# optimusride/altro-cpp

Measured on AMD Instinct MI355X. Metric: trajectories solved/sec (AL-iLQR to tol), unicycle 101 knots, batched, higher is better.
Workload: dtype f64; 1 GPU; BASELINE configs[2]: batch 4096/GPU unicycle kTurn90 (n=3, m=2, 101 knots), goal + control-bound constraints, full AL loop, default SolverOptions; batch_per_gpu=4096, global_batch=4096, knot_points=101, parallelism=instance-sharded x1 (no data-path collective; RCCL all_gather of result records), device=AMD Radeon Graphics, cus=256

## Files before the change

altro-cpp_amd/csrc/altro_common.hpp:

```cpp
#pragma once

#include <algorithm>
#include <atomic>
#include <cstddef>
#include <initializer_list>
#include <string>
#include <vector>

#include "../../include/altro_hip.h"

namespace altro_hip {

constexpr int kMaxConPerKnot = 4;
constexpr int kMaxClasses = 8;
constexpr int kMaxCostGroups = 8;
#ifndef ALTRO_LS_LANES
#define ALTRO_LS_LANES 20
#endif
constexpr int kLineSearchLanes = ALTRO_LS_LANES;
constexpr int kHistFields = 8;
constexpr int kMaxRuns = 16;
constexpr int kMaxFastCircles = 3;
constexpr int kMaxSharedPool = 128;
constexpr int kParPerKnot = 2;
// ... 366 lines not shown
  ALTRO_HD int total() const { return raw() + fwd_block_pad_bytes((long long)raw() * (long long)sizeof(T)) / (int)sizeof(T); }
};
template <class T>
struct FusedLds {
  FwdLds<T> blk;
  int N, nm, npool;
  static constexpr int kE = (int)sizeof(T), kD = (int)sizeof(double);
  ALTRO_HD int oPool() const { return blk.total() * kE; }
  ALTRO_HD int oXch() const { return oPool() + blk.padv(npool) * kE; }
  ALTRO_HD int oFlags() const { return oXch() + 2 * kSyncFused * nm * kBlock * kE; }
  ALTRO_HD int oGrad() const { return oFlags() + 2 * kBlock * (int)sizeof(int); }
  ALTRO_HD int oFh() const { return oGrad() + kBlock * kD; }
  ALTRO_HD int oJunk() const { return oFh() + kFhWords * kD; }
  ALTRO_HD int oActive() const { return oJunk() + kBlock * kD; }
  ALTRO_HD int oFf() const { return oActive() + 2 * kD; }
  ALTRO_HD int oCand() const { return oFf() + kFfWords * kD; }
  ALTRO_HD int oKD2() const { return oCand() + (N + 1) * kLineSearchLanes * nm * kE; }
  ALTRO_HD int oFh2() const { return oKD2() + (blk.nKD + kBlock) * kE; }
  ALTRO_HD int oAlpha() const { return oFh2() + kFh2Words * kD; }
  ALTRO_HD int oSync() const { return oAlpha() + kLineSearchLanes * kD; }
  ALTRO_HD int oCost() const { return oSync() + kSyWords * (int)sizeof(int); }
  ALTRO_HD int oCvalAhead() const { return oCost() + ((N + 2) & ~1) * kE; }
  ALTRO_HD int used() const { return oCvalAhead() + blk.rowsP() * kE; }
  ALTRO_HD size_t bytes() const { return (size_t)used() + 8 * kD + (size_t)(N + 4 - ((N + 2) & ~1)) * kE; }
};

inline int ChainClaimLocal(int device, int delta) {
  static std::atomic<int> n[64];
  std::atomic<int>& c = n[device >= 0 && device < 64 ? device : 63];
  if (delta == 0) return c.load();
  return c.fetch_add(delta) + delta;
}
using ChainClaimFn = int (*)(int, int);
inline ChainClaimFn& ChainClaimHook() {
  static ChainClaimFn fn = &ChainClaimLocal;
  return fn;
}
inline int ChainClaim(int device, int delta) { return ChainClaimHook()(device, delta); }

class EngineBase {
 public:
  virtual ~EngineBase() {}
  virtual altro_status Upload(const ProblemSpec& spec, std::string* err) = 0;
  virtual altro_status SetInitialState(const ProblemSpec& spec, std::string* err) = 0;
  virtual altro_status SetTrajectory(const ProblemSpec& spec, std::string* err) = 0;
  virtual altro_status SetStep(float hstep) = 0;
// ... 82 lines not shown
```

altro-cpp_amd/csrc/altro_engine.hpp:

```cpp
#pragma once

#include <algorithm>
#include <atomic>
#include <chrono>
#include <cmath>
#include <cstdio>
#include <cstdlib>
#include <cstring>
#include <limits>
#include <map>
#include <string>
#include <thread>
#include <type_traits>
#include <vector>

#include "altro_devmem.hpp"
#include "altro_kernels.hpp"
#include "altro_problem.hpp"

namespace altro_hip {

#define ALTRO_HIP_CHECK(expr)                                                                  \
  do {                                                                                         \
    hipError_t e_ = (expr);                                                                    \
// ... 17 lines not shown
struct Switches {
  struct OptInt {
    bool set = false;
    int v = 0;
  };
  bool poison_on = false;
  unsigned poison_pattern = 0;
  int poison_mix = 0;
  OptInt persist_at;
  bool twin = true;
  bool segments = true;
  OptInt chains;
  OptInt fwd_per_wave;
  int fwd_src = kFwdSrcAuto;
  int sweep_loop = -1;
  OptInt loop_per_cu;
  int cand_front = 6;
  bool twin_debug = false;
  bool twin_debug_all = false;
  int twin_depth = kTwinDefaultDepth;
  int twin_min = tw_min_share(kTwinDefaultMin);
  int twin_spread = kTwinDefaultSpread;
  int twin_misclaim = 0;
  const char* sweep_log = nullptr;
  bool loop_log = false;
  bool force_valu_backward = false, force_coop_backward = false;
  bool dense_expansions = true;
  int spec_mode = kSpecAuto;
  bool fast_forward = false;
  bool begin_merged = true;
  bool no_fused = false;

  static bool NotZero(const char* e) { return !(e && atoi(e) == 0); }
  static bool Is(const char* e, const char* what) { return e && std::strcmp(e, what) == 0; }
  Switches() {
    auto env = [](const char* name) { return std::getenv(name); };
    auto number = [&](const char* name) {
      const char* e = env(name);
      return e ? OptInt{true, atoi(e)} : OptInt{};
    };
    if (const char* e = env("ALTRO_HIP_DEBUG_POISON")) {
      poison_on = true;
      poison_pattern = (unsigned)strtoul(e, nullptr, 16);
      poison_mix = std::strchr(e, ',') != nullptr;
    }
    persist_at = number("ALTRO_HIP_PERSIST_AT");
    twin = NotZero(env("ALTRO_HIP_TWIN"));
    segments = NotZero(env("ALTRO_HIP_SEGMENTS"));
    chains = number("ALTRO_HIP_CHAINS");
    if (chains.set) chains.v = std::max(1, std::min(kMaxSweepChains, chains.v));
    fwd_per_wave = number("ALTRO_HIP_FWD_PER_WAVE");
    if (const char* e = env("ALTRO_HIP_FWD_SRC")) fwd_src = Is(e, "global") ? kFwdSrcGlobal : kFwdSrcOther;
    if (const char* e = env("ALTRO_HIP_SWEEP_LOOP")) sweep_loop = NotZero(e) ? 1 : 0;
    loop_per_cu = number("ALTRO_HIP_LOOP_PER_CU");
    if (const char* e = env("ALTRO_HIP_CAND_FRONT")) cand_front = std::max(0, std::min(kLineSearchLanes - 1, atoi(e)));
    twin_debug = env("ALTRO_HIP_TWIN_DEBUG") != nullptr;
    twin_debug_all = Is(env("ALTRO_HIP_TWIN_DEBUG"), "all");
    if (const char* e = env("ALTRO_HIP_TWIN_DEPTH")) twin_depth = std::max(1, std::min(kTwinMaxDepth, atoi(e)));
    if (const char* e = env("ALTRO_HIP_TWIN_MIN")) twin_min = tw_min_share(atoi(e));
    if (const char* e = env("ALTRO_HIP_TWIN_SPREAD")) twin_spread = std::max(0, std::min(kTwinMaxSpread, atoi(e)));
    if (const char* e = env("ALTRO_HIP_TWIN_MISCLAIM")) twin_misclaim = std::max(0, atoi(e));
    sweep_log = env("ALTRO_HIP_SWEEP_LOG");
    loop_log = env("ALTRO_HIP_LOOP_LOG") != nullptr;
    force_valu_backward = Is(env("ALTRO_HIP_BACKWARD"), "valu");
    force_coop_backward = Is(env("ALTRO_HIP_BACKWARD"), "coop");
    dense_expansions = env("ALTRO_HIP_NO_DENSE_EXPANSIONS") == nullptr;
    const char* spec = env("ALTRO_HIP_SPECULATION");
    spec_mode = Is(spec, "off") ? (int)kSpecOff : Is(spec, "free") ? (int)kSpecFree : Is(spec, "wave") ? (int)kSpecWave : kSpecAuto;
    fast_forward = env("ALTRO_HIP_FAST_FORWARD_STALLS") != nullptr;
    begin_merged = !Is(env("ALTRO_HIP_BEGIN_SOLVE"), "split");
    no_fused = env("ALTRO_HIP_NO_FUSED_SWEEP") != nullptr;
  }
};

inline DevOpts ToDevOpts(const altro_options& o) {
  DevOpts d{};
  d.max_iterations_total = o.max_iterations_total;
  d.max_iterations_outer = o.max_iterations_outer;
  d.max_iterations_inner = o.max_iterations_inner;
  d.bp_reg_fail_threshold = o.bp_reg_fail_threshold;
  d.check_forwardpass_bounds = o.check_forwardpass_bounds;
  d.line_search_max_iterations = o.line_search_max_iterations;
  d.reset_duals = o.reset_duals;
  d.cost_tolerance = o.cost_tolerance;
// ... 2480 lines not shown
        A.act_list = up_.d_merged;
        A.act_count = merged_count;
        timing_.launches += 1;
      }
      A.host_count = nullptr;
      A.next_list = nullptr;
      A.next_count = nullptr;
      PoisonLds();
      if (r.prof) {
        r.fused_ev = r.nev;
        hipEventRecord(ProfEvent(r.nev++), stream_);
      }
      bool circles = false;
      for (int k = 0; k < pd_.nruns; ++k)
        circles = circles || pd_.runs[k].fast == kFastC || pd_.runs[k].fast == kFastCB || pd_.runs[k].fast == kFastBC;
      int* const out = r.loop_launched ? up_.d_loop_ctl + kLwWords : hm_.d_counter.get() + r.max_sweeps + 2;
      const int spec = sw_.spec_mode == kSpecAuto ? (circles ? (int)kSpecWave : (int)kSpecFree) : sw_.spec_mode;
      TwinCtl tw{};
      if (up_.twin_cap > 0 && !A.hist && !r.d.fast_forward_stalls) {
        if (!twin_box_clean_)
          hipMemsetAsync(up_.d_twin_box, 0, TwinBoxWords() * sizeof(unsigned long long), stream_);
        const int min_share = any_split ? std::max(sw_.twin_min, kTwinSegMin) : sw_.twin_min;
        const int pool = std::min(up_.twin_cap, std::max(ninst, num_cus_ - ninst));
        tw = TwinCtl{up_.d_twin_box, up_.d_twin_box + (size_t)2 * up_.twin_cap * kTwWords, ninst, up_.twin_cap, Bp_ - up_.twin_cap, kTwinLag, sw_.twin_debug ? 1 : 0,
                     pool, any_split ? 1 : sw_.twin_depth, min_share, sw_.twin_spread, sw_.twin_misclaim};
      }
      const dim3 g(ninst + (tw.base > 0 ? tw.npool : 0)), b3(kFwdWaves * kBlock), b4((kFwdWaves + 1) * kBlock);
      timing_.twin_workgroups = tw.base > 0 ? (int)g.x - ninst : 0;
      ForEachFusedVariant([&](auto v) {
        using V = decltype(v);
        if (V::circles == circles && V::spec == spec && V::segments == any_split)
          hipLaunchKernelGGL((k_sweep_fused<T, M, V::circles, V::spec, V::segments>), g, V::spec == kSpecOff ? b3 : b4, fused_lds_bytes_,
                             stream_, A, up_.d_pd, pd_, r.d, r.mode, 1, out, tw);
      });
      if (r.prof) hipEventRecord(ProfEvent(r.nev++), stream_);
      r.persistent_launched = true;
      timing_.launches += 1;
    }
    return ALTRO_OK;
  }
  altro_status WaitForDevice(SolveRun& r) {
    if (r.nap_ok && !r.nap)
      r.nap = r.loop_launched || std::chrono::duration<double, std::micro>(std::chrono::steady_clock::now() - r.t0).count() > kHostNapAfterUs;
    if (r.nap && tail_ev_) {
      ALTRO_HIP_CHECK(hipEventRecord(tail_ev_, stream_));
      for (;;) {
        const hipError_t q = hipEventQuery(tail_ev_);
        if (q == hipSuccess) break;
        if (q != hipErrorNotReady) ALTRO_HIP_CHECK(q);
        std::this_thread::sleep_for(std::chrono::microseconds(20));
        timing_.host_naps += 1;
      }
    }
    for (int c = 1; c < r.C; ++c) ALTRO_HIP_CHECK(hipStreamSynchronize(r.chain[c].st));
    ALTRO_HIP_CHECK(hipStreamSynchronize(stream_));
    ALTRO_HIP_CHECK(hipGetLastError());
// ... 37 lines not shown
        ALTRO_HIP_CHECK(CopySync(extra, hm_.d_counter.get() + r.max_sweeps + 2, sizeof(extra), hipMemcpyDeviceToHost));
      }
      timing_.twin_handovers = extra[kRwHandovers];
      timing_.twin_claims = extra[kRwClaims];
      timing_.fused_workgroup_iterations = extra[kRwGroupLoops];
      if (r.seg_on && sw_.twin_debug) {
        int cur[kMaxChains] = {0};
        ALTRO_HIP_CHECK(CopySync(cur, up_.d_seg_cursor, sizeof(cur), hipMemcpyDeviceToHost));
        fprintf(stderr, "segments: shadow columns used per chain %d %d %d %d (of %d each), persistent launch over <= %d slots, longest own chain %d, longest workgroup %d\n",
                cur[0], cur[1], cur[2], cur[3], r.seg_capc, (int)timing_.twin_workgroups, extra[kRwChainLoops], extra[kRwGroupLoops]);
      }
      if (up_.twin_cap > 0 && sw_.twin_debug) ALTRO_TRY(DumpTwinMailboxes());
      if (extra[kRwSyncErr] != 0) {
        err_ = "k_sweep_fused: a forward wave gave up waiting for its sequence word (software synchronisation)";
        return ALTRO_HIP_ERROR;
      }
      timing_.fused_sweeps = extra[kRwChainLoops];
      timing_.fused_instance_iterations = extra[kRwUnits];
      sweeps = std::max(sweeps, extra[kRwSweeps]);
    }
    timing_.sweeps = sweeps;
    return ALTRO_OK;
  }
  size_t TwinBoxWords() const { return (size_t)2 * up_.twin_cap * (kTwWords + 1); }
  altro_status DumpTwinMailboxes() {
    const int nbox = 2 * up_.twin_cap;
    std::vector<unsigned long long> box((size_t)nbox * kTwWords);
    ALTRO_HIP_CHECK(CopySync(box.data(), up_.d_twin_box, box.size() * sizeof(unsigned long long), hipMemcpyDeviceToHost));
    int hist[4] = {0, 0, 0, 0}, why[8] = {0}, by_depth[kTwinMaxDepth + 2] = {0};
    unsigned long long t0 = ~0ull;
    for (int s = 0; s < up_.twin_cap; ++s)
      if (box[(size_t)s * kTwWords + kTwStamp + kTsPStart]) t0 = std::min(t0, box[(size_t)s * kTwWords + kTwStamp + kTsPStart]);
    auto us_of = [&](const unsigned long long* ts, int i) { return ts[i] ? (double)(long long)(ts[i] - t0) * 0.01 : -1.0; };
    int shown = 0;
    double last_commit = 0, last_pend = 0, last_tstart = 0, last_leave = 0;
    int s_commit = -1, s_pend = -1;
    for (int s = 0; s < nbox; ++s) {
      const unsigned long long* w = &box[(size_t)s * kTwWords];
      const unsigned long long* ts = w + kTwStamp;
      auto us = [&](int i) { return us_of(ts, i); };
      if (s >= up_.twin_cap && w[kTwClaim] != 0) {
        hist[w[kTwHand] & 3]++;
        by_depth[std::min<unsigned long long>(w[kTwGen], kTwinMaxDepth + 1)]++;
        const int limit = timing_.twin_claims <= 48 || sw_.twin_debug_all ? 1 : 8;
        if ((shown++ % limit) == 0)
          fprintf(stderr, "  segment %4d depth %d inst %d from %d: it %d..%d hand %d | start %.0f go %.0f cloned %.0f first %.0f snap %.0f claimed %.0f "
                  "done %.0f (loops %llu) verdict %.0f handed %.0f commit %.0f\n", s, (int)w[kTwGen], (int)w[kTwInst] - 1, (int)w[kTwPred] - 1,
                  (int)(w[kTwClaim] >> 32), (int)w[kTwEnd], (int)(w[kTwHand] & 3), us(kTsTStart), us(kTsTGo), us(kTsTCloned), us(kTsTFirst), us(kTsPSnap),
                  us(kTsPClaim), us(kTsTDone), ts[kTsTLoops], us(kTsTVerdict), us(kTsPHand), us(kTsTCommit));
      }
      if (sw_.twin_debug_all && s < up_.twin_cap && ts[kTsPStart] != 0)
        fprintf(stderr, "  primary %4d: start %.0f snap %.0f claimed %.0f handed %.0f end %.0f\n", s, us(kTsPStart), us(kTsPSnap), us(kTsPClaim),
                us(kTsPHand), us(kTsPEnd));
      if (sw_.twin_debug_all && s >= up_.twin_cap && w[kTwClaim] == 0 && ts[kTsTIdleEnd] != 0)
        fprintf(stderr, "  idle %4d: start %.0f left %.0f\n", s, us(kTsTStart), us(kTsTIdleEnd));
      if (w[kTwWhy] != 0) {
        why[w[kTwWhy] & 7]++;
        if (why[w[kTwWhy] & 7] <= 3)
          fprintf(stderr, "  worker %d refused its successor: why %d at it_inner %d (claim start %d)\n", s, (int)(w[kTwWhy] & 7),
                  (int)((w[kTwWhy] >> 8) & 0xffff), (int)((w[kTwWhy] >> 24) & 0xffff));
      }
      if (us(kTsTCommit) > last_commit) { last_commit = us(kTsTCommit); s_commit = s; }
      if (us(kTsPEnd) > last_pend) { last_pend = us(kTsPEnd); s_pend = s; }
      last_leave = std::max(last_leave, us(kTsPHand));
      last_tstart = std::max(last_tstart, us(kTsTStart));
    }
    fprintf(stderr, "twin timeline: last commit %.0f us (mailbox %d), last primary that finished by itself %.0f us (slot %d), last hand-over %.0f us, "
            "last pool start %.0f us\n", last_commit, s_commit, last_pend, s_pend, last_leave, last_tstart);
    fprintf(stderr, "twin mailboxes: pool %d claims %d confirmed joints %d | segments by depth: 1: %d 2: %d 3: %d 4: %d 5: %d | hand word: open %d ok %d refused %d "
            "revoked %d | refusals: streak broke %d, passed %d, counters %d, rho %d, drho %d, break since snapshot %d\n", (int)timing_.twin_workgroups,
            (int)timing_.twin_claims, (int)timing_.twin_handovers, by_depth[1], by_depth[2], by_depth[3], by_depth[4], by_depth[5], hist[0], hist[1], hist[2],
            hist[3], why[1], why[2], why[3], why[4], why[5], why[6]);
    return ALTRO_OK;
  }
  void AccountProfile(SolveRun& r) {
    float ms = 0, fused_ms = 0;
    hipEventElapsedTime(&ms, prof_ev_[0], prof_ev_[1]);
    timing_.init_ms = ms;
// ... 103 lines not shown
  altro_desc desc_;
  int B_ = 0, Bp_ = 0, N_ = 0;
  bool uploaded_ = false;
  bool last_mode_ilqr_ = false;
  DevOpts last_opts_{};
  bool ctg_fresh_ = false;
  bool ctg_replayable_ = false;
  ProblemDesc pd_{};
  DevArrays<T> A_{};
  void SegArrays(DevArrays<T>& A) const {
    A.seg_end = up_.seg.end; A.seg_next = up_.seg.next; A.seg_flag = up_.seg.flag; A.seg_streak = up_.seg.streak;
    A.seg_tot0 = up_.seg.tot0; A.seg_rho0 = up_.seg.rho0; A.seg_drho0 = up_.seg.drho0;
  }
  int seg_col0_ = 0, seg_parts_ = 4;
  const Switches sw_;
  int seg_below_pct_ = 65;
  bool mfma_offsets_ok_ = false;
  bool kdg_ = false;
  bool rg_ = false;
  int fwd_per_wave_ = kBlock / kLineSearchLanes;
  size_t fwd_lds_bytes_ = 0, fwd_shared_bytes_ = 0, fwd_per_inst_bytes_ = 0;
  int num_cus_ = 256;
  bool twin_box_clean_ = false;
  static constexpr int kMaxChains = kMaxSweepChains;
  static constexpr int kDefaultChains = 4;
  bool counted_chained_ = false;
  long long chain_overlap_ticks_ = 0;
  int chains_ = 1;
  int chain_size_ = 0;
  hipStream_t chain_stream_[kMaxChains] = {};
  hipEvent_t chain_ev_[kMaxChains] = {};
  hipEvent_t start_ev_ = nullptr;
  hipEvent_t tail_ev_ = nullptr;
  static constexpr int kHostNapMinBatch = 256;
  static constexpr unsigned kHostSpinsBeforeNap = 400;
  static constexpr double kHostNapAfterUs = 500.0;
  bool host_wait_backoff_ = true;
  int loop_per_cu_ = 0;
  size_t loop_lds_bytes_ = 0;
  static constexpr int lanes_per_wave() { return kBlock / kLineSearchLanes; }
  template <int SRC>
  static const void* LoopKernel() {
    if constexpr (kMfmaBackward && (SRC != kSrcGlb || kRgEligible))
      return reinterpret_cast<const void*>(&k_sweep_loop<T, M, SRC>);
    else
      return nullptr;
// ... 32 lines not shown
```

altro-cpp_amd/csrc/altro_kernels.hpp:

```cpp
#pragma once

#include <type_traits>

#include "altro_device.hpp"

namespace altro_hip {

constexpr int kFwdWaves = 3;
constexpr int kEAheadToErrWord = -7;
constexpr int kFwdSpinLimit = 1 << 22;
template <int kDummy>
__global__ __launch_bounds__(256) void k_poison_columns(unsigned* arr, unsigned rows, unsigned Bp, unsigned col0, unsigned ncols,
                                                         unsigned words, unsigned pattern, int mix) {
  const size_t per_row = (size_t)ncols * words, total = (size_t)rows * per_row;
  for (size_t i = (size_t)blockIdx.x * 256 + threadIdx.x; i < total; i += (size_t)gridDim.x * 256) {
    const size_t r = i / per_row, w = i - r * per_row;
    arr[(r * Bp + col0) * words + w] = mix ? (pattern ^ ((unsigned)i * 2654435761u)) : pattern;
  }
}
template <int kDummy>
__global__ __launch_bounds__(256) void k_poison_lds(unsigned pattern, int words, int mix, int* sink) {
  extern __shared__ unsigned poison_smem[];
  for (int i = threadIdx.x; i < words; i += 256) poison_smem[i] = mix ? (pattern ^ ((unsigned)i * 2654435761u)) : pattern;
  __syncthreads();
// ... 3276 lines not shown
      using RR = Rec<RS, n, m>;
      store_rec_as<T, RS, R::EP, RR::EP, R::eE>(RECP((RS*)A.EXP, k, RR::EP), E);
    }
    toff = (toff + ((cnt + kBlock - 1) / kBlock) * kBlock) % nthreads;
  }
}

enum SpecMode { kSpecOff = 0, kSpecWave = 1, kSpecFree = 3 };
ALTRO_DEV constexpr bool spec_has_wave4(int spec) { return spec == kSpecWave || spec == kSpecFree; }

struct TwinCtl {
  unsigned long long* box;
  unsigned long long* state;
  int base;
  int cap;
  int col0;
  int lag;
  int debug;
  int npool;
  int depth;
  int min_share;
  int spread;
  int misclaim;
};
enum TwinStamp { kTsPStart = 0, kTsPSnap = 1, kTsPClaim = 2, kTsPHand = 3, kTsPLoopsAtSnap = 4, kTsTStart = 5, kTsTGo = 6, kTsTCloned = 7,
                 kTsTFirst = 8, kTsTDone = 9, kTsTVerdict = 10, kTsTCommit = 11, kTsTLoops = 12, kTsPEnd = 13,
                 kTsTIdleEnd = 14  };
enum TwinWord {
  kTwSeq = 0,
  kTwSnap = 1,
  kTwProg = 7,
  kTwSucc = 8,
  kTwEnd = 9,
  kTwGen = 10,
  kTwInst = 11,
  kTwClaim = 12,
  kTwClaimRho = 13,
  kTwClaimDrho = 14,
  kTwClaimSnap = 15,
  kTwHand = 16,
  kTwHandLoops = 17,
  kTwWhy = 18,
  kTwPred = 19,
  kTwStamp = 20,
  kTwWords = 40
};
constexpr unsigned long long kTwOk = 1, kTwRefused = 2, kTwRevoked = 3;
constexpr unsigned long long kTwSuccId = 0xffffull;
constexpr unsigned long long kTwFrozen = 1ull << 32;
constexpr unsigned long long kTwsSnap = 1, kTwsClosed = 2, kTwsLocked = 4, kTwsFull = 8, kTwsBusy = 16;
// ... 34 lines not shown
  return __hip_atomic_compare_exchange_strong(p, &expect, v, __ATOMIC_RELAXED, __ATOMIC_RELAXED, __HIP_MEMORY_SCOPE_AGENT);
}
ALTRO_DEV unsigned long long tw_bits(double x) { return (unsigned long long)__double_as_longlong(x); }
ALTRO_DEV double tw_dbl(unsigned long long x) { return __longlong_as_double((long long)x); }
ALTRO_DEV int tw_remaining(const DevOpts& o, unsigned long long prog, int end_inner) {
  const int it_in = (int)(prog >> 32), it_tot = (int)(prog & 0xffffffffull);
  if (end_inner > 0) return end_inner - it_in;
  const int r1 = o.max_iterations_inner - it_in, r2 = o.max_iterations_total - it_tot;
  return r1 < r2 ? r1 : r2;
}
ALTRO_HD int tw_keep(int R, int lag) { return (R + lag) / 2 + 1; }
ALTRO_HD bool tw_claimable(int R, int lag, int min_share) { return R >= 2 * min_share && R - tw_keep(R, lag) >= min_share; }
ALTRO_DEV void tw_cancel_chain(const TwinCtl& tw, unsigned long long* box) {
  unsigned long long nx = __hip_atomic_fetch_or(box + kTwSucc, kTwFrozen, __ATOMIC_RELAXED, __HIP_MEMORY_SCOPE_AGENT) & kTwSuccId;
  for (int guard = 0; nx != 0 && nx <= (unsigned long long)(2 * tw.cap) && guard < (2 << kTwinMaxDepth); ++guard) {
    const int id = (int)nx - 1;
    unsigned long long* sb = tw.box + (size_t)id * kTwWords;
    nx = __hip_atomic_fetch_or(sb + kTwSucc, kTwFrozen, __ATOMIC_RELAXED, __HIP_MEMORY_SCOPE_AGENT) & kTwSuccId;
    tw_cas(sb + kTwHand, 0ull, kTwRefused);
    __hip_atomic_fetch_or(tw.state + id, kTwsClosed, __ATOMIC_RELAXED, __HIP_MEMORY_SCOPE_AGENT);
  }
}

template <class T>
struct TailCtx {
  const DevArrays<T>& A;
  const ProblemDesc* pd;
  const DevOpts& o;
  const TwinCtl& tw;
  int* sweeps_out;
  double* ff;
  int tid;
};
struct TwinWorker {
  unsigned long long* box = nullptr;
  int slot = -1;
  bool is_twin = false;
  int streak = 0;
  int break_total = -1;
  unsigned long long ver = 0;
  bool closed = false;
  bool shown = false;
  unsigned long long succ = 0, claim = 0;
  unsigned long long peek = 0;
  bool full = false;
  bool confirmed = false;
// ... 145 lines not shown
ALTRO_DEV void tw_show(const TwinCtl& tw, TwinWorker& w, unsigned long long cnt, double rho, double drho, int b_real, int loops) {
  ++w.ver;
  unsigned long long* buf = w.box + kTwSnap + 3 * (w.ver & 1);
  tw_store(buf, cnt);
  tw_store(buf + 1, tw_bits(rho));
  tw_store(buf + 2, tw_bits(drho));
  tw_store(w.box + kTwInst, (unsigned long long)(unsigned)(b_real + 1));
  __builtin_amdgcn_fence(__ATOMIC_RELEASE, "agent");
  tw_order();
  tw_store(w.box + kTwSeq, w.ver);
  tw_order();
  __hip_atomic_fetch_or(tw.state + w.slot, kTwsSnap, __ATOMIC_RELAXED, __HIP_MEMORY_SCOPE_AGENT);
  w.shown = true;
  w.stamp(tw, kTsPSnap);
  w.stamp(tw, kTsPLoopsAtSnap, loops);
}
template <class T, class M, bool SEG>
ALTRO_DEV bool tw_enter_clone(const TailCtx<T>& C, TwinWorker& w, int tslot, long long tstart_clock, int nthreads, int* b,
                              int* b_real) {
  const DevArrays<T>& A = C.A;
  const TwinCtl& tw = C.tw;
  double* const ff = C.ff;
  const int tid = C.tid;
  const int src_id = (int)ff[kFfClaimSource];
  if (src_id < 0) return false;
  w.slot = tw.cap + tslot;
  w.box = tw.box + (size_t)w.slot * kTwWords;
  *b_real = (int)ff[kFfClaimInst];
  const int b_src = src_id < tw.cap ? instance_of_slot(A, src_id, 0) : tw.col0 + (src_id - tw.cap);
  if (tid == 0) {
    w.stamp(tw, kTsTStart, tstart_clock);
    w.stamp(tw, kTsTGo);
  }
  const int bT = tw.col0 + tslot;
  copy_column<T, M>(A, C.pd, (unsigned)b_src, (unsigned)bT, kColTwinClone, tid, nthreads);
  if (tid == 0) {
    if (SEG && A.seg_end) {
      A.seg_end[bT] = kSegNoEnd;
      A.seg_next[bT] = -1;
      A.seg_flag[bT] = 0;
      A.seg_streak[bT] = 2;
    }
    A.cost_prev[bT] = A.cost_cur[bT];
    A.it_inner[bT] = (int)ff[kFfClaimItInner];
    A.it_total[bT] = (int)ff[kFfClaimItTotal];
    A.rho_reg[bT] = ff[kFfClaimRho];
    A.drho[bT] = ff[kFfClaimDrho];
  }
  *b = bT;
  __syncthreads();
  if (tid == 0) w.stamp(tw, kTsTCloned);
  if (tid == 0) {
    ff[kFfClaimOpen] = tw_load(w.box + kTwHand) == 0 ? 1.0 : 0.0;
    if (ff[kFfClaimOpen] == 0.0) w.close(tw);
    else if ((int)((tw_load(w.box + kTwSucc) >> 16) & 0xffffull) < tw.depth) {
      const unsigned long long cnt = ((unsigned long long)(unsigned)(int)ff[kFfClaimItInner] << 32) | (unsigned long long)(unsigned)(int)ff[kFfClaimItTotal];
      tw_store(w.box + kTwProg, cnt);
      tw_show(tw, w, cnt, ff[kFfClaimRho], ff[kFfClaimDrho], *b_real, 0);
    }
  }
  __syncthreads();
  return ff[kFfClaimOpen] != 0.0;
}

template <class T>
ALTRO_DEV void fused_adopt_spec(const DevArrays<T>& A, int b, T* sKDf, const T* sKD2, int nKD, double* fh, const double* fh2,
                                int tid, int nthreads) {
  for (int i = tid; i < nKD; i += nthreads) sKDf[i] = sKD2[i];
  if (tid == 0) {
    double h[6];
    h[0] = fh2[kFhDV0]; h[1] = fh2[kFhDV1]; h[2] = fh2[kFhRho]; h[3] = fh2[kFhDrho]; h[4] = fh2[kFhRegLog];
    fh[kFhDV0] = h[0];
    fh[kFhDV1] = h[1];
    fh[kFhRho] = h[2];
    fh[kFhDrho] = h[3];
    A.dV0[b] = h[0];
    A.dV1[b] = h[1];
    A.reg_log[b] = h[4];
    A.rho_reg[b] = h[2];
    A.drho[b] = h[3];
  }
}

template <class T, class M, bool WAVE4>
ALTRO_DEV void fused_expand_ahead(const DevArrays<T>& A, const ProblemDesc* pd, const FwdLds<T>& L, T* sm, T* sPool, T* sCost,
// ... 156 lines not shown
    w.close(tw);
    w.closed = true;
    w.stamp(tw, kTsPHand);
    C.ff[kFfHandResult] = res;
    C.ff[kFfLoopsBefore] = (double)w.loops0;
  }
  __syncthreads();
  return C.ff[kFfHandResult];
}
template <class T, class M>
ALTRO_DEV bool tw_commit(const TailCtx<T>& C, TwinWorker& w, int loops, int b, int b_real, int nthreads) {
  const TwinCtl& tw = C.tw;
  double* const ff = C.ff;
  if (C.tid == 0) {
    w.stamp(tw, kTsTDone);
    w.stamp(tw, kTsTLoops, loops);
    const unsigned long long h = w.confirmed ? kTwOk : tw_await_verdict(C, w);
    if (!w.closed) tw_cancel_chain(tw, w.box);
    w.close(tw);
    ff[kFfLoopsBefore] = (double)w.loops0;
    ff[kFfCommitOk] = h == kTwOk ? 1.0 : 0.0;
  }
  __syncthreads();
  if (ff[kFfCommitOk] == 0.0) return false;
  w.loops0 = (int)ff[kFfLoopsBefore];
  copy_column<T, M>(C.A, C.pd, (unsigned)b, (unsigned)b_real, kColTwinCommit, C.tid, nthreads);
  if (C.tid == 0) w.stamp(tw, kTsTCommit);
  return true;
}
#ifdef ALTRO_STAMPS
ALTRO_DEV void fused_stamp_summary(int b, int loops, int spec_iters) {
  const double c = 1.0 / spec_iters;
  const double ca = 1.0 / loops;
  printf("STAMPS (instance %d): %d iterations, %d adopted (speculated); per adopted iteration, shader-clock cycles:\n"
         "  E %.0f | take-over %.0f | forward pass (wave 0) %.0f | barrier behind F (wave 0 waits) %.0f | whole iteration %.0f\n"
         "  rollout wave: knot loop %.0f, wait A+S %.0f, phase 2 %.0f\n"
         "  cost wave: knot loop + wait A %.0f, selection %.0f, phase 2 + wait V %.0f, phase 3 %.0f\n"
         "  auxiliary wave: knot loop %.0f | fourth wave: speculative backward pass %.0f (only passes of armed iterations)\n"
         "  take-over: copy + hand-over (wave 0) %.0f, running cost (wave 1) %.0f | E alone, waves 0..3: %.0f %.0f %.0f %.0f | E ahead (wave 0) %.0f\n",
         b, loops, spec_iters, c * g_stamp_acc[9], c * g_stamp_acc[10], c * g_stamp_acc[11], c * g_stamp_acc[12], c * g_stamp_acc[14],
         ca * g_stamp_acc[0], ca * g_stamp_acc[1], ca * g_stamp_acc[2], ca * g_stamp_acc[3], ca * g_stamp_acc[4], ca * g_stamp_acc[5],
         ca * g_stamp_acc[6], ca * g_stamp_acc[7], c * g_stamp_acc[8], c * g_stamp_acc[16], c * g_stamp_acc[15],
         c * g_stamp_acc[17], c * g_stamp_acc[18], c * g_stamp_acc[19], c * g_stamp_acc[20], c * g_stamp_acc[21]);
}
#endif

template <class T>
// ... 12 lines not shown
  T* alpha_tab;
  int* sync_words;
  T* sCost;
  T* sCvalAhead;
  ALTRO_DEV FusedSmem(unsigned char* raw, const FwdLds<T>& L, const FusedLds<T>& F)
      : sm(reinterpret_cast<T*>(raw)), sKDf(sm + L.nX + L.nU), sPool(reinterpret_cast<T*>(raw + F.oPool())),
        xch(reinterpret_cast<T*>(raw + F.oXch())), fh(reinterpret_cast<double*>(raw + F.oFh())),
        fused_junk((int)(reinterpret_cast<T*>(raw + F.oJunk()) - sKDf)), active_flag(reinterpret_cast<int*>(raw + F.oActive())),
        ff(reinterpret_cast<double*>(raw + F.oFf())), sCand(reinterpret_cast<T*>(raw + F.oCand())),
        sKD2(reinterpret_cast<T*>(raw + F.oKD2())), fh2(reinterpret_cast<double*>(raw + F.oFh2())),
        alpha_tab(reinterpret_cast<T*>(raw + F.oAlpha())), sync_words(reinterpret_cast<int*>(raw + F.oSync())),
        sCost(reinterpret_cast<T*>(raw + F.oCost())), sCvalAhead(reinterpret_cast<T*>(raw + F.oCvalAhead())) {}
};
template <class T>
ALTRO_DEV void fused_init_lds(const FusedSmem<T>& S, const DevOpts& o, int tid) {
  if (tid < kSyWords) S.sync_words[tid] = 0;
  if (tid < kLineSearchLanes) {
    T alpha = T(1);
    for (int i = 0; i < tid; ++i) alpha /= T(o.line_search_decrease_factor);
    S.alpha_tab[tid] = alpha;
  }
}

template <class T, class M, bool CIRC, int SPEC, bool SEG = false>
__global__ __launch_bounds__((spec_has_wave4(SPEC) ? kFwdWaves + 1 : kFwdWaves) * kBlock) void k_sweep_fused(
    DevArrays<T> A, const ProblemDesc* __restrict__ pdg, const ProblemDesc pd_arg, DevOpts o, int mode, int persistent,
    int* sweeps_out, TwinCtl tw) {
  constexpr int kThreads = (spec_has_wave4(SPEC) ? kFwdWaves + 1 : kFwdWaves) * kBlock;
  constexpr bool kWave4 = spec_has_wave4(SPEC), kSoft = SPEC == kSpecFree;
  using R = Rec<T, M::n, M::m>;
  constexpr int nm = M::n + M::m;
  extern __shared__ __align__(16) unsigned char smem_raw[];
  const ProblemDesc* pd = &pd_arg;
  const int tid = threadIdx.x, wave = tid >> 6, lane = tid & 63;
  if (blockIdx.x == 0 && tid == 0) publish_count(A);
  TwinWorker w;
  w.is_twin = tw.base > 0 && (int)blockIdx.x >= tw.base;
  const int tslot = w.is_twin ? (int)blockIdx.x - tw.base : -1;
  w.slot = w.is_twin ? -1 : (int)blockIdx.x;
  int b_real = w.is_twin ? -1 : instance_of_slot(A, w.slot, 0);
  if (!w.is_twin && b_real < 0) return;
  if (w.is_twin && (tslot >= tw.npool || tslot >= tw.cap || !persistent)) return;
  if (!w.is_twin && tw.base > 0 && w.slot < tw.cap && persistent) w.box = tw.box + (size_t)w.slot * kTwWords;
  int b = b_real;
  const int N = A.N;
  const unsigned Bp = A.Bp;
  const FwdLds<T> L{(N + 1) * R::nP, N * R::mP, N * R::KP, pd->total_rows, pd->nslots, R::V};
  const FusedSmem<T> S(smem_raw, L, FusedLds<T>{L, N, nm, pd->npool});
  FwdSpec<T> spec{S.sKD2, L.nKD, S.fh2, S.fh2 + kFhSpecRho, false};
  fused_init_lds(S, o, tid);
  const TailCtx<T> C{A, pd, o, tw, sweeps_out, S.ff, tid};
  bool adopt = false;
  StallWatch stall;
  int skipped = 0;
  int loops = 0;
  bool e_done = false;
#ifdef ALTRO_STAMPS
  if (tid < 32) g_stamp_acc[tid] = 0;
  int spec_iters = 0;
#endif
  const long long tstart_clock = tw.debug ? wall_clock64() : 0;
  if (tid == 0 && !w.is_twin) w.stamp(tw, kTsPStart);
  if (w.is_twin) {
    if (wave == 0) tw_find_work(C, tw.cap + tslot, lane);
    __syncthreads();
    if (!tw_enter_clone<T, M, SEG>(C, w, tslot, tstart_clock, kThreads, &b, &b_real)) {
      if (tid == 0 && tw.debug) {
        unsigned long long* own = tw.box + (size_t)(tw.cap + tslot) * kTwWords + kTwStamp;
        tw_store(own + kTsTStart, (unsigned long long)tstart_clock);
        tw_store(own + kTsTIdleEnd, (unsigned long long)wall_clock64());
      }
      return;
    }
  }
  if (wave == 2 && lane == 0) {
    S.ff[kFfInitCost] = A.initial_cost[b];
    S.ff[kFfNeedInitCost] = A.need_init_cost[b] ? 1.0 : 0.0;
  }
  for (;;) {
    const long long st_it = ALTRO_STAMP_T0();
    if (w.box && tid == 0 && !w.closed && !w.full && (w.is_twin || w.shown)) w.peek = tw_load(w.box + kTwSucc);
    if (loops == 0) {
      forward2_stage<T, M>(A, pd, L, smem_raw, S.sPool, 1, 0, tid, kThreads, kKdNone, true, -1, b);
      __syncthreads();
    }
    const CtxL<T> CE(A, b, S.sPool, S.sm + L.nX + L.nU + L.nKD + 2 * L.rowsP(), S.sm + L.nX + L.nU + L.nKD,
                     S.sm + L.nX + L.nU + L.nKD + L.rowsP());
    if (!e_done) {
      expansion_from_lds<T, M>(A, pd, CE, S.sm, S.sm + L.nX, S.sCost, b, tid, kThreads);
      if (adopt) ALTRO_STAMP_ADD(17 + wave, st_it);
      if (SPEC && adopt) lds_barrier(); else __syncthreads();
    }
    if (wave == 0 && adopt) ALTRO_STAMP_ADD(9, st_it);
    const long long st_b = ALTRO_STAMP_T0();

// ... 9 lines not shown
    if (wave == 0 && adopt) ALTRO_STAMP_ADD(10, st_b);
    const long long st_f = ALTRO_STAMP_T0();
    const bool st_adopted = adopt;
    spec.armed = armed;
    forward2_body<T, M, true, kSrcLds, CIRC, kSoft, false>(A, pdg, pd, o, mode, 0, 1, smem_raw, S.fh, S.active_flag, S.sCand, S.ff,
                                                    kWave4 ? &spec : nullptr, S.alpha_tab,
                                                    FwdSync<kSoft>{S.sync_words, loops * kFwdSeqStride}, S.sCost, S.fh,
                                                    S.sync_words + kSyEAhead0, persistent ? (kWave4 ? 3 : 2) : 0, loops + 1, b);
    ++loops;
    if (wave == 0 && st_adopted) ALTRO_STAMP_ADD(11, st_f);
    const long long st_x = ALTRO_STAMP_T0();
    if (persistent && wave != 1 && reinterpret_cast<const int*>(S.xch)[1] == 0) {
      fused_expand_ahead<T, M, kWave4>(A, pd, L, S.sm, S.sPool, S.sCost, S.sCvalAhead, S.sync_words, b, wave, lane, loops);
      if (wave == 0 && st_adopted) ALTRO_STAMP_ADD(21, st_x);
    }
    if (SPEC) lds_barrier(); else __syncthreads();
    if (wave == 0 && st_adopted) ALTRO_STAMP_ADD(12, st_x);
#ifdef ALTRO_STAMPS
    if (st_adopted) {
      ++spec_iters;
      if (wave == 0) ALTRO_STAMP_ADD(14, st_it);
    }
#endif
    if (!persistent || *S.active_flag == 0) break;
    e_done = S.ff[kFfRejected] != 0.0 && S.ff[kFfInnerDone] == 0.0;
    if (e_done)
      for (int r = tid; r < pd->total_rows; r += kThreads) A.cval[(unsigned)r * Bp + (unsigned)b] = S.sCvalAhead[r];
    if (kWave4)
      adopt = armed && S.fh2[kFhSpecOk] != 0.0 && S.ff[kFfRejected] != 0.0 && S.ff[kFfInnerDone] == 0.0 && S.ff[kFfRho] == S.fh2[kFhSpecRho] &&
              S.ff[kFfDrho] == S.fh2[kFhSpecDrho];
    if (o.fast_forward_stalls) skipped += fused_fast_forward(C, stall, b);
    if (SEG && A.seg_end) {
      if (tid == 0) fused_seg_joint(C, b);
      if (SPEC && adopt) lds_barrier(); else __syncthreads();
      if (S.ff[kFfSegLeave] != 0.0) break;
    }
    if (w.box) tw_bookkeeping<T, SEG>(C, w, loops, b, b_real);
    if (SPEC && adopt) lds_barrier(); else __syncthreads();
    if (w.box) {
      const double act = S.ff[kFfTwinAction];
      if (act == 1.0) {
        if (tid == 0) w.close(tw);
        return;
      }
      if (act == 2.0) {
        const double res = tw_hand_over(C, w, loops);
        if (res == 3.0) {
          fused_report<T, SEG, kSoft>(C, b_real, S.sync_words, (int)S.ff[kFfLoopsBefore] + loops + skipped, loops, skipped);
          return;
        }
        if (res == 1.0) return;
      }
    }
  }
  if (w.is_twin) {
    if (!tw_commit<T, M>(C, w, loops, b, b_real, kThreads)) return;
    b = b_real;
  } else if (w.box && tid == 0 && !w.closed) {
    tw_cancel_chain(tw, w.box);
    w.close(tw);
    w.stamp(tw, kTsPEnd);
  }
#ifdef ALTRO_STAMPS
  __syncthreads();
  if (tid == 0 && spec_iters > 60 && loops > 100) fused_stamp_summary(b, loops, spec_iters);
#endif
  for (int i = tid; i < N * R::KP; i += kThreads) {
    const int k = i / R::KP, e = i - k * R::KP;
    using RS = rec_scalar_t<T, M>;
    if (e < (Rec<RS, M::n, M::m>::KP)) RECP((RS*)A.KD, k, (Rec<RS, M::n, M::m>::KP))[e] = (RS)S.sKDf[i];
  }
  fused_report<T, SEG, kSoft>(C, b_real, S.sync_words, w.loops0 + loops + skipped, loops, skipped);
}


template <class T, class M>
__global__ __launch_bounds__(kBlock) void k_seg_fixup(DevArrays<T> A, const ProblemDesc* __restrict__ pd) {
  const int b = blockIdx.x, tid = threadIdx.x;
  if (b >= A.B) return;
  int cur = b;
  for (int guard = 0; guard < 4096; ++guard) {
    const int nx = A.seg_next[cur];
    if (!(A.seg_flag[cur] & kSegRetired) || nx < 0 || (A.seg_flag[nx] & kSegCancelled)) break;
    cur = nx;
  }
  if (cur == b) return;
  copy_column<T, M>(A, pd, (unsigned)cur, (unsigned)b, kColSegFixup, tid, kBlock);
}

enum LoopWord {
  kLwFinished = 0,
  kLwTail = 1,
  kLwUnits = 2,
  kLwMaxLoops = 3,
  kLwGroups = 4,
  kLwTicks = 8,
  kLwCursor = 16,
// ... 1019 lines not shown
```

altro-cpp_amd/csrc/inst_unicycle_f64.hip:

```cpp
#include "altro_engine.hpp"
namespace altro_hip {
EngineBase* MakeEngineUnicycleF64(const altro_desc& d, std::string* err) { return MakeEngineImpl<double, UnicycleM>(d, err); }
}

extern "C" int altro_twin_policy(int R, int lag, int asked_min, int* keep, int* claimable, int* see_claim) {
  const int min_share = altro_hip::tw_min_share(asked_min);
  if (keep) *keep = altro_hip::tw_keep(R, lag);
  if (claimable) *claimable = altro_hip::tw_claimable(R, lag, min_share) ? 1 : 0;
  if (see_claim) *see_claim = altro_hip::kTwinSeeClaim;
  return min_share;
}
```

Before: 684,400 trajectories/s.

## Run fused sweep as persistent ticket-driven workers over primary and twin jobs

```diff
diff --git a/altro-cpp_amd/csrc/altro_common.hpp b/altro-cpp_amd/csrc/altro_common.hpp
--- a/altro-cpp_amd/csrc/altro_common.hpp
+++ b/altro-cpp_amd/csrc/altro_common.hpp
@@ -412,6 +412,7 @@
   ALTRO_HD int oCost() const { return oSync() + kSyWords * (int)sizeof(int); }
   ALTRO_HD int oCvalAhead() const { return oCost() + ((N + 2) & ~1) * kE; }
   ALTRO_HD int used() const { return oCvalAhead() + blk.rowsP() * kE; }
+  ALTRO_HD int oTicket() const { return used(); }
   ALTRO_HD size_t bytes() const { return (size_t)used() + 8 * kD + (size_t)(N + 4 - ((N + 2) & ~1)) * kE; }
 };
 
diff --git a/altro-cpp_amd/csrc/altro_engine.hpp b/altro-cpp_amd/csrc/altro_engine.hpp
--- a/altro-cpp_amd/csrc/altro_engine.hpp
+++ b/altro-cpp_amd/csrc/altro_engine.hpp
@@ -63,6 +63,7 @@
   int twin_min = tw_min_share(kTwinDefaultMin);
   int twin_spread = kTwinDefaultSpread;
   int twin_misclaim = 0;
+  int tail_workers = kTailWorkersDefault;
   const char* sweep_log = nullptr;
   bool loop_log = false;
   bool force_valu_backward = false, force_coop_backward = false;
@@ -101,6 +102,7 @@
     if (const char* e = env("ALTRO_HIP_TWIN_MIN")) twin_min = tw_min_share(atoi(e));
     if (const char* e = env("ALTRO_HIP_TWIN_SPREAD")) twin_spread = std::max(0, std::min(kTwinMaxSpread, atoi(e)));
     if (const char* e = env("ALTRO_HIP_TWIN_MISCLAIM")) twin_misclaim = std::max(0, atoi(e));
+    if (const char* e = env("ALTRO_HIP_TAIL_WORKERS")) tail_workers = std::max(0, atoi(e));
     sweep_log = env("ALTRO_HIP_SWEEP_LOG");
     loop_log = env("ALTRO_HIP_LOOP_LOG") != nullptr;
     force_valu_backward = Is(env("ALTRO_HIP_BACKWARD"), "valu");
@@ -2627,16 +2629,24 @@
           hipMemsetAsync(up_.d_twin_box, 0, TwinBoxWords() * sizeof(unsigned long long), stream_);
         const int min_share = any_split ? std::max(sw_.twin_min, kTwinSegMin) : sw_.twin_min;
         const int pool = std::min(up_.twin_cap, std::max(ninst, num_cus_ - ninst));
-        tw = TwinCtl{up_.d_twin_box, up_.d_twin_box + (size_t)2 * up_.twin_cap * kTwWords, ninst, up_.twin_cap, Bp_ - up_.twin_cap, kTwinLag, sw_.twin_debug ? 1 : 0,
-                     pool, any_split ? 1 : sw_.twin_depth, min_share, sw_.twin_spread, sw_.twin_misclaim};
-      }
-      const dim3 g(ninst + (tw.base > 0 ? tw.npool : 0)), b3(kFwdWaves * kBlock), b4((kFwdWaves + 1) * kBlock);
-      timing_.twin_workgroups = tw.base > 0 ? (int)g.x - ninst : 0;
+        unsigned long long* const state = up_.d_twin_box + (size_t)2 * up_.twin_cap * kTwWords;
+        tw = TwinCtl{up_.d_twin_box, state, ninst, up_.twin_cap, Bp_ - up_.twin_cap, kTwinLag, sw_.twin_debug ? 1 : 0,
+                     pool, any_split ? 1 : sw_.twin_depth, min_share, sw_.twin_spread, sw_.twin_misclaim,
+                     0, reinterpret_cast<int*>(state + (size_t)2 * up_.twin_cap)};
+      }
+      const int npool = tw.base > 0 ? tw.npool : 0;
+      const dim3 b3(kFwdWaves * kBlock), b4((kFwdWaves + 1) * kBlock);
+      timing_.twin_workgroups = npool;
       ForEachFusedVariant([&](auto v) {
         using V = decltype(v);
-        if (V::circles == circles && V::spec == spec && V::segments == any_split)
-          hipLaunchKernelGGL((k_sweep_fused<T, M, V::circles, V::spec, V::segments>), g, V::spec == kSpecOff ? b3 : b4, fused_lds_bytes_,
-                             stream_, A, up_.d_pd, pd_, r.d, r.mode, 1, out, tw);
+        if (V::circles == circles && V::spec == spec && V::segments == any_split) {
+          const dim3 blk = V::spec == kSpecOff ? b3 : b4;
+          if (tw.base > 0 && sw_.tail_workers != 0)
+            tw.workers = tail_worker_count(ninst, npool, num_cus_, FusedPerCu(V::Fn(), (int)blk.x), sw_.tail_workers);
+          const dim3 g(tail_grid(ninst, npool, tw.workers));
+          hipLaunchKernelGGL((k_sweep_fused<T, M, V::circles, V::spec, V::segments>), g, blk, fused_lds_bytes_, stream_, A, up_.d_pd, pd_,
+                             r.d, r.mode, 1, out, tw);
+        }
       });
       if (r.prof) hipEventRecord(ProfEvent(r.nev++), stream_);
       r.persistent_launched = true;
@@ -2720,7 +2730,17 @@
     timing_.sweeps = sweeps;
     return ALTRO_OK;
   }
-  size_t TwinBoxWords() const { return (size_t)2 * up_.twin_cap * (kTwWords + 1); }
+  size_t TwinBoxWords() const { return (size_t)2 * up_.twin_cap * (kTwWords + 1) + 1; }
+  int FusedPerCu(const void* fn, int threads) {
+    if (fn != fused_per_cu_fn_ || fused_lds_bytes_ != fused_per_cu_lds_) {
+      int n = 0;
+      if (hipOccupancyMaxActiveBlocksPerMultiprocessor(&n, fn, threads, fused_lds_bytes_) != hipSuccess) n = 0;
+      fused_per_cu_ = n;
+      fused_per_cu_fn_ = fn;
+      fused_per_cu_lds_ = fused_lds_bytes_;
+    }
+    return fused_per_cu_;
+  }
   altro_status DumpTwinMailboxes() {
     const int nbox = 2 * up_.twin_cap;
     std::vector<unsigned long long> box((size_t)nbox * kTwWords);
@@ -2743,15 +2763,15 @@
         const int limit = timing_.twin_claims <= 48 || sw_.twin_debug_all ? 1 : 8;
         if ((shown++ % limit) == 0)
           fprintf(stderr, "  segment %4d depth %d inst %d from %d: it %d..%d hand %d | start %.0f go %.0f cloned %.0f first %.0f snap %.0f claimed %.0f "
-                  "done %.0f (loops %llu) verdict %.0f handed %.0f commit %.0f\n", s, (int)w[kTwGen], (int)w[kTwInst] - 1, (int)w[kTwPred] - 1,
+                  "done %.0f (loops %llu) verdict %.0f handed %.0f commit %.0f | xcd %d worker %d\n", s, (int)w[kTwGen], (int)w[kTwInst] - 1, (int)w[kTwPred] - 1,
                   (int)(w[kTwClaim] >> 32), (int)w[kTwEnd], (int)(w[kTwHand] & 3), us(kTsTStart), us(kTsTGo), us(kTsTCloned), us(kTsTFirst), us(kTsPSnap),
-                  us(kTsPClaim), us(kTsTDone), ts[kTsTLoops], us(kTsTVerdict), us(kTsPHand), us(kTsTCommit));
+                  us(kTsPClaim), us(kTsTDone), ts[kTsTLoops], us(kTsTVerdict), us(kTsPHand), us(kTsTCommit), (int)ts[kTsXcd] - 1, (int)ts[kTsWorker] - 1);
       }
       if (sw_.twin_debug_all && s < up_.twin_cap && ts[kTsPStart] != 0)
-        fprintf(stderr, "  primary %4d: start %.0f snap %.0f claimed %.0f handed %.0f end %.0f\n", s, us(kTsPStart), us(kTsPSnap), us(kTsPClaim),
-                us(kTsPHand), us(kTsPEnd));
+        fprintf(stderr, "  primary %4d: start %.0f snap %.0f claimed %.0f handed %.0f end %.0f | xcd %d worker %d\n", s, us(kTsPStart), us(kTsPSnap), us(kTsPClaim),
+                us(kTsPHand), us(kTsPEnd), (int)ts[kTsXcd] - 1, (int)ts[kTsWorker] - 1);
       if (sw_.twin_debug_all && s >= up_.twin_cap && w[kTwClaim] == 0 && ts[kTsTIdleEnd] != 0)
-        fprintf(stderr, "  idle %4d: start %.0f left %.0f\n", s, us(kTsTStart), us(kTsTIdleEnd));
+        fprintf(stderr, "  idle %4d: start %.0f left %.0f | xcd %d worker %d\n", s, us(kTsTStart), us(kTsTIdleEnd), (int)ts[kTsXcd] - 1, (int)ts[kTsWorker] - 1);
       if (w[kTwWhy] != 0) {
         why[w[kTwWhy] & 7]++;
         if (why[w[kTwWhy] & 7] <= 3)
@@ -2901,6 +2921,9 @@
   size_t fwd_lds_bytes_ = 0, fwd_shared_bytes_ = 0, fwd_per_inst_bytes_ = 0;
   int num_cus_ = 256;
   bool twin_box_clean_ = false;
+  const void* fused_per_cu_fn_ = nullptr;
+  size_t fused_per_cu_lds_ = 0;
+  int fused_per_cu_ = 0;
   static constexpr int kMaxChains = kMaxSweepChains;
   static constexpr int kDefaultChains = 4;
   bool counted_chained_ = false;
diff --git a/altro-cpp_amd/csrc/altro_kernels.hpp b/altro-cpp_amd/csrc/altro_kernels.hpp
--- a/altro-cpp_amd/csrc/altro_kernels.hpp
+++ b/altro-cpp_amd/csrc/altro_kernels.hpp
@@ -3322,10 +3322,30 @@
   int min_share;
   int spread;
   int misclaim;
+  int workers;
+  int* tickets;
 };
+enum TailTicket { kTkPrimary = 0, kTkPool = 1, kTkWords = 2 };
+#ifndef ALTRO_TAIL_WORKERS
+#define ALTRO_TAIL_WORKERS -1
+#endif
+constexpr int kTailWorkersDefault = ALTRO_TAIL_WORKERS;
+ALTRO_HD int tail_worker_count(int ninst, int npool, int cus, int per_cu, int asked) {
+  const int jobs = ninst + npool, room = cus * per_cu;
+  if (asked == 0 || room <= 0) return 0;
+  int n = jobs < room ? jobs : room;
+  if (asked > 0 && asked < n) n = asked;
+  return n;
+}
+ALTRO_HD int tail_grid(int ninst, int npool, int workers) { return workers > 0 ? workers : ninst + npool; }
+ALTRO_HD int tail_block_of_ticket(int kind, int ticket, int ninst, int npool) {
+  if (kind == kTkPrimary) return ticket < ninst ? ticket : -1;
+  return ticket < npool ? ninst + ticket : -1;
+}
 enum TwinStamp { kTsPStart = 0, kTsPSnap = 1, kTsPClaim = 2, kTsPHand = 3, kTsPLoopsAtSnap = 4, kTsTStart = 5, kTsTGo = 6, kTsTCloned = 7,
                  kTsTFirst = 8, kTsTDone = 9, kTsTVerdict = 10, kTsTCommit = 11, kTsTLoops = 12, kTsPEnd = 13,
-                 kTsTIdleEnd = 14  };
+                 kTsTIdleEnd = 14 ,
+                 kTsXcd = 15 , kTsWorker = 16  };
 enum TwinWord {
   kTwSeq = 0,
   kTwSnap = 1,
@@ -3406,6 +3426,7 @@
   }
 }
 
+ALTRO_DEV bool wg_uniform(bool c) { return __builtin_amdgcn_readfirstlane(c ? 1 : 0) != 0; }
 template <class T>
 struct TailCtx {
   const DevArrays<T>& A;
@@ -3597,7 +3618,7 @@
   const TwinCtl& tw = C.tw;
   double* const ff = C.ff;
   const int tid = C.tid;
-  const int src_id = (int)ff[kFfClaimSource];
+  const int src_id = __builtin_amdgcn_readfirstlane((int)ff[kFfClaimSource]);
   if (src_id < 0) return false;
   w.slot = tw.cap + tslot;
   w.box = tw.box + (size_t)w.slot * kTwWords;
@@ -3635,7 +3656,7 @@
     }
   }
   __syncthreads();
-  return ff[kFfClaimOpen] != 0.0;
+  return wg_uniform(ff[kFfClaimOpen] != 0.0);
 }
 
 template <class T>
@@ -3838,7 +3859,7 @@
     ff[kFfCommitOk] = h == kTwOk ? 1.0 : 0.0;
   }
   __syncthreads();
-  if (ff[kFfCommitOk] == 0.0) return false;
+  if (wg_uniform(ff[kFfCommitOk] == 0.0)) return false;
   w.loops0 = (int)ff[kFfLoopsBefore];
   copy_column<T, M>(C.A, C.pd, (unsigned)b, (unsigned)b_real, kColTwinCommit, C.tid, nthreads);
   if (C.tid == 0) w.stamp(tw, kTsTCommit);
@@ -3897,25 +3918,23 @@
   }
 }
 
-template <class T, class M, bool CIRC, int SPEC, bool SEG = false>
-__global__ __launch_bounds__((spec_has_wave4(SPEC) ? kFwdWaves + 1 : kFwdWaves) * kBlock) void k_sweep_fused(
-    DevArrays<T> A, const ProblemDesc* __restrict__ pdg, const ProblemDesc pd_arg, DevOpts o, int mode, int persistent,
-    int* sweeps_out, TwinCtl tw) {
+template <class T, class M, bool CIRC, int SPEC, bool SEG>
+ALTRO_DEV bool fused_job(const DevArrays<T>& A, const ProblemDesc* __restrict__ pdg, const ProblemDesc* pd, const DevOpts& o, int mode,
+                         int persistent, int* sweeps_out, const TwinCtl& tw, unsigned char* smem_raw, int vblock) {
   constexpr int kThreads = (spec_has_wave4(SPEC) ? kFwdWaves + 1 : kFwdWaves) * kBlock;
   constexpr bool kWave4 = spec_has_wave4(SPEC), kSoft = SPEC == kSpecFree;
   using R = Rec<T, M::n, M::m>;
   constexpr int nm = M::n + M::m;
-  extern __shared__ __align__(16) unsigned char smem_raw[];
-  const ProblemDesc* pd = &pd_arg;
-  const int tid = threadIdx.x, wave = tid >> 6, lane = tid & 63;
-  if (blockIdx.x == 0 && tid == 0) publish_count(A);
+  int tid = threadIdx.x;
+  asm volatile("" : "+v"(tid));
+  const int wave = tid >> 6, lane = tid & 63;
   TwinWorker w;
-  w.is_twin = tw.base > 0 && (int)blockIdx.x >= tw.base;
-  const int tslot = w.is_twin ? (int)blockIdx.x - tw.base : -1;
-  w.slot = w.is_twin ? -1 : (int)blockIdx.x;
+  w.is_twin = tw.base > 0 && vblock >= tw.base;
+  const int tslot = w.is_twin ? vblock - tw.base : -1;
+  w.slot = w.is_twin ? -1 : vblock;
   int b_real = w.is_twin ? -1 : instance_of_slot(A, w.slot, 0);
-  if (!w.is_twin && b_real < 0) return;
-  if (w.is_twin && (tslot >= tw.npool || tslot >= tw.cap || !persistent)) return;
+  if (!w.is_twin && b_real < 0) return false;
+  if (w.is_twin && (tslot >= tw.npool || tslot >= tw.cap || !persistent)) return false;
   if (!w.is_twin && tw.base > 0 && w.slot < tw.cap && persistent) w.box = tw.box + (size_t)w.slot * kTwWords;
   int b = b_real;
   const int N = A.N;
@@ -3936,6 +3955,12 @@
 #endif
   const long long tstart_clock = tw.debug ? wall_clock64() : 0;
   if (tid == 0 && !w.is_twin) w.stamp(tw, kTsPStart);
+  const unsigned xcc = tw.debug ? (__builtin_amdgcn_s_getreg(20 | (0 << 6) | (3 << 11)) & 15u) : 0u;
+  if (tid == 0 && tw.debug && tw.base > 0 && (w.is_twin || w.box)) {
+    unsigned long long* own = (w.is_twin ? tw.box + (size_t)(tw.cap + tslot) * kTwWords : w.box) + kTwStamp;
+    tw_store(own + kTsXcd, (unsigned long long)xcc + 1ull);
+    tw_store(own + kTsWorker, (unsigned long long)blockIdx.x + 1ull);
+  }
   if (w.is_twin) {
     if (wave == 0) tw_find_work(C, tw.cap + tslot, lane);
     __syncthreads();
@@ -3945,7 +3970,7 @@
         tw_store(own + kTsTStart, (unsigned long long)tstart_clock);
         tw_store(own + kTsTIdleEnd, (unsigned long long)wall_clock64());
       }
-      return;
+      return wg_uniform(S.ff[kFfClaimSource] < 0.0);
     }
   }
   if (wave == 2 && lane == 0) {
@@ -4001,7 +4026,7 @@
       if (wave == 0) ALTRO_STAMP_ADD(14, st_it);
     }
 #endif
-    if (!persistent || *S.active_flag == 0) break;
+    if (!persistent || wg_uniform(*S.active_flag == 0)) break;
     e_done = S.ff[kFfRejected] != 0.0 && S.ff[kFfInnerDone] == 0.0;
     if (e_done)
       for (int r = tid; r < pd->total_rows; r += kThreads) A.cval[(unsigned)r * Bp + (unsigned)b] = S.sCvalAhead[r];
@@ -4012,28 +4037,28 @@
     if (SEG && A.seg_end) {
       if (tid == 0) fused_seg_joint(C, b);
       if (SPEC && adopt) lds_barrier(); else __syncthreads();
-      if (S.ff[kFfSegLeave] != 0.0) break;
+      if (wg_uniform(S.ff[kFfSegLeave] != 0.0)) break;
     }
     if (w.box) tw_bookkeeping<T, SEG>(C, w, loops, b, b_real);
     if (SPEC && adopt) lds_barrier(); else __syncthreads();
     if (w.box) {
-      const double act = S.ff[kFfTwinAction];
-      if (act == 1.0) {
+      const int act = __builtin_amdgcn_readfirstlane((int)S.ff[kFfTwinAction]);
+      if (act == 1) {
         if (tid == 0) w.close(tw);
-        return;
-      }
-      if (act == 2.0) {
-        const double res = tw_hand_over(C, w, loops);
-        if (res == 3.0) {
+        return false;
+      }
+      if (act == 2) {
+        const int res = __builtin_amdgcn_readfirstlane((int)tw_hand_over(C, w, loops));
+        if (res == 3) {
           fused_report<T, SEG, kSoft>(C, b_real, S.sync_words, (int)S.ff[kFfLoopsBefore] + loops + skipped, loops, skipped);
-          return;
-        }
-        if (res == 1.0) return;
+          return false;
+        }
+        if (res == 1) return false;
       }
     }
   }
   if (w.is_twin) {
-    if (!tw_commit<T, M>(C, w, loops, b, b_real, kThreads)) return;
+    if (!tw_commit<T, M>(C, w, loops, b, b_real, kThreads)) return false;
     b = b_real;
   } else if (w.box && tid == 0 && !w.closed) {
     tw_cancel_chain(tw, w.box);
@@ -4050,8 +4075,46 @@
     if (e < (Rec<RS, M::n, M::m>::KP)) RECP((RS*)A.KD, k, (Rec<RS, M::n, M::m>::KP))[e] = (RS)S.sKDf[i];
   }
   fused_report<T, SEG, kSoft>(C, b_real, S.sync_words, w.loops0 + loops + skipped, loops, skipped);
-}
-
+  return false;
+}
+
+template <class T, class M, bool CIRC, int SPEC, bool SEG = false>
+__global__ __launch_bounds__((spec_has_wave4(SPEC) ? kFwdWaves + 1 : kFwdWaves) * kBlock) void k_sweep_fused(
+    DevArrays<T> A, const ProblemDesc* __restrict__ pdg, const ProblemDesc pd_arg, DevOpts o, int mode, int persistent,
+    int* sweeps_out, TwinCtl tw) {
+  using R = Rec<T, M::n, M::m>;
+  extern __shared__ __align__(16) unsigned char smem_raw[];
+  const ProblemDesc* pd = &pd_arg;
+  if (blockIdx.x == 0 && threadIdx.x == 0) publish_count(A);
+  const bool workers = tw.workers > 0 && persistent;
+  const int N = A.N;
+  const FusedLds<T> F{FwdLds<T>{(N + 1) * R::nP, N * R::mP, N * R::KP, pd->total_rows, pd->nslots, R::V}, N, M::n + M::m, pd->npool};
+  int* const ticket = reinterpret_cast<int*>(smem_raw + F.oTicket());
+  double* const ff = reinterpret_cast<double*>(smem_raw + F.oFf());
+  double* const fh = reinterpret_cast<double*>(smem_raw + F.oFh());
+  double* const fh2 = reinterpret_cast<double*>(smem_raw + F.oFh2());
+  bool pool_phase = false;
+  for (;;) {
+    int vb = (int)blockIdx.x;
+    if (workers) {
+      __syncthreads();
+      if (threadIdx.x == 0) {
+        int t = -1;
+        if (!pool_phase) t = tail_block_of_ticket(kTkPrimary, atomicAdd(tw.tickets + kTkPrimary, 1), tw.base, tw.npool);
+        if (t < 0) t = tail_block_of_ticket(kTkPool, atomicAdd(tw.tickets + kTkPool, 1), tw.base, tw.npool);
+        *ticket = t;
+      }
+      if (threadIdx.x < kFfWords) ff[threadIdx.x] = 0.0;
+      if (threadIdx.x < kFhWords) fh[threadIdx.x] = 0.0;
+      if (threadIdx.x < kFh2Words) fh2[threadIdx.x] = 0.0;
+      __syncthreads();
+      vb = __builtin_amdgcn_readfirstlane(*ticket);
+      if (vb < 0) break;
+      pool_phase = vb >= tw.base;
+    }
+    if (fused_job<T, M, CIRC, SPEC, SEG>(A, pdg, pd, o, mode, persistent, sweeps_out, tw, smem_raw, vb) || !workers) break;
+  }
+}
 
 template <class T, class M>
 __global__ __launch_bounds__(kBlock) void k_seg_fixup(DevArrays<T> A, const ProblemDesc* __restrict__ pd) {
diff --git a/altro-cpp_amd/csrc/inst_unicycle_f64.hip b/altro-cpp_amd/csrc/inst_unicycle_f64.hip
--- a/altro-cpp_amd/csrc/inst_unicycle_f64.hip
+++ b/altro-cpp_amd/csrc/inst_unicycle_f64.hip
@@ -10,3 +10,10 @@
   if (see_claim) *see_claim = altro_hip::kTwinSeeClaim;
   return min_share;
 }
+
+extern "C" int altro_tail_tickets(int ninst, int npool, int cus, int per_cu, int asked, int kind, int ticket, int* workers, int* block) {
+  const int w = altro_hip::tail_worker_count(ninst, npool, cus, per_cu, asked);
+  if (workers) *workers = w;
+  if (block) *block = altro_hip::tail_block_of_ticket(kind, ticket, ninst, npool);
+  return altro_hip::tail_grid(ninst, npool, w);
+}
```

After: 715,000 trajectories/s, median of 6. 4.5% higher.
